# X-PLUG/Youku-mPLUG

Measured on NVIDIA H100. Metric: video-text samples/sec (pretrain 1.3B, 8f x 224^2), higher is better.
Workload: dtype bf16

## Files before the change

### youku-mplug_b200/csrc/gemm_wgmma.cu

```cuda
#include <cuda.h>

#include "common.h"
#include "philox.cuh"
#include "ptx.cuh"
#include "wgmma.cuh"

namespace ymp {

constexpr int BM = 128;
constexpr int BK = 64;
constexpr int WGMMA_K = 16;
constexpr int GEMM_THREADS = 3 * 128;
constexpr int A_STAGE_BYTES = BM * BK * 2;

struct GemmKParams {
  void* D;
  const __nv_bfloat16* bias;
  const void* residual;
  __nv_bfloat16* aux_out;
  const __nv_bfloat16* aux_in;
  int M, N, K;
  int ldd, ldr;
  int a_mn, b_mn;
  int act, out_f32, accumulate, split_k;
  int kb_per_split;
  int res_row_mod;
  int d_row_block, d_row_stride;
  int res_f32;
  int n_fast;
  float alpha;
  int im2col_T, im2col_N, im2col_Wp;
  DropSpec drop;
  int has_drop;
};

template <int BN>
struct GemmCfg {
  static constexpr int NSTAGE = (BN == 256) ? 4 : 6;
  static constexpr int B_STAGE_BYTES = BN * BK * 2;
  static constexpr int STAGE_BYTES = A_STAGE_BYTES + B_STAGE_BYTES;
  static constexpr int STG_LD = BN + 4;
  static_assert(BM * STG_LD * 4 <= NSTAGE * STAGE_BYTES, "epilogue staging reuses the operand ring");
  static constexpr int SMEM_BYTES = NSTAGE * STAGE_BYTES + 256 + 1024;
};

template <int BN>
struct EpiCfg {
  static constexpr int TPR = BN / 8;
  static constexpr int RPP = 256 / TPR;
  static constexpr int GROUP = 4;
  static_assert(BM % (RPP * GROUP) == 0, "row groups tile BM");
};

__device__ __forceinline__ uint2 ld_bf16x4(const __nv_bfloat16* p) { return __ldg(reinterpret_cast<const uint2*>(p)); }
__device__ __forceinline__ void st_bf16x4(__nv_bfloat16* p, const float* f) {
  *reinterpret_cast<uint2*>(p) = make_uint2(pack_bf16(f[0], f[1]), pack_bf16(f[2], f[3]));
}

struct EpiIn {
  uint32_t res[8];
  uint32_t aux[4];
};
__device__ __forceinline__ void epilogue_fetch(const GemmKParams& p, int row, const int (&col)[2], bool full, EpiIn& in) {
  if (row >= p.M || !full) return;
  if (p.aux_in) {
#pragma unroll
    for (int q = 0; q < 2; ++q) {
      const uint2 a = ld_bf16x4(p.aux_in + (size_t)row * p.ldd + col[q]);
      in.aux[2 * q] = a.x; in.aux[2 * q + 1] = a.y;
    }
  }
  if (p.residual) {
    const int rrow = p.res_row_mod ? row % p.res_row_mod : row;
#pragma unroll
    for (int q = 0; q < 2; ++q) {
      if (p.res_f32) {
        const float4 a = __ldg(reinterpret_cast<const float4*>(reinterpret_cast<const float*>(p.residual) + (size_t)rrow * p.ldr + col[q]));
        in.res[4 * q] = __float_as_uint(a.x); in.res[4 * q + 1] = __float_as_uint(a.y);
        in.res[4 * q + 2] = __float_as_uint(a.z); in.res[4 * q + 3] = __float_as_uint(a.w);
      } else {
        const uint2 a = ld_bf16x4(reinterpret_cast<const __nv_bfloat16*>(p.residual) + (size_t)rrow * p.ldr + col[q]);
        in.res[2 * q] = a.x; in.res[2 * q + 1] = a.y;
      }
    }
  }
}

template <bool DROP>
__device__ __forceinline__ void epilogue_row(const GemmKParams& p, float (&v)[8], int row, const int (&col)[2], bool full,
                                             const uint32_t (&bias)[4], const EpiIn& in, const DropState& ds) {
  if (row >= p.M) return;
  const int drow = p.d_row_block ? (row / p.d_row_block) * p.d_row_stride + row % p.d_row_block : row;
  const int rrow = p.res_row_mod ? row % p.res_row_mod : row;
  if (p.alpha != 1.0f) {
#pragma unroll
    for (int i = 0; i < 8; ++i) v[i] = v[i] * p.alpha;
  }

  if (full) {
    if (p.bias) {
#pragma unroll
      for (int i = 0; i < 4; ++i) { v[2 * i] += bf16_lo(bias[i]); v[2 * i + 1] += bf16_hi(bias[i]); }
    }
    const size_t off[2] = {(size_t)row * p.ldd + col[0], (size_t)row * p.ldd + col[1]};
    const size_t doff[2] = {(size_t)drow * p.ldd + col[0], (size_t)drow * p.ldd + col[1]};
    if (p.aux_in) {
#pragma unroll
      for (int i = 0; i < 4; ++i) { v[2 * i] *= bf16_lo(in.aux[i]); v[2 * i + 1] *= bf16_hi(in.aux[i]); }
    } else if (p.act == YMP_ACT_GELU_ERF) {
      if (p.aux_out) {
        float x[8], d[8];
#pragma unroll
        for (int i = 0; i < 8; ++i) x[i] = v[i];
        gelu_erf_both_x8(x, v, d);
        st_bf16x4(p.aux_out + off[0], d);
        st_bf16x4(p.aux_out + off[1], d + 4);
      } else {
        float x[8];
#pragma unroll
        for (int i = 0; i < 8; ++i) x[i] = v[i];
        gelu_erf_x8(x, v);
      }
    } else if (p.act == YMP_ACT_GELU_TANH) {
      if (p.aux_out) {
        float d[8];
#pragma unroll
        for (int i = 0; i < 8; ++i) v[i] = gelu_tanh_both(v[i], d[i]);
        st_bf16x4(p.aux_out + off[0], d);
        st_bf16x4(p.aux_out + off[1], d + 4);
      } else {
#pragma unroll
        for (int i = 0; i < 8; ++i) v[i] = gelu_tanh(v[i]);
      }
    } else if (p.aux_out) {
      st_bf16x4(p.aux_out + off[0], v);
      st_bf16x4(p.aux_out + off[1], v + 4);
    }
    if constexpr (DROP) {
#pragma unroll
      for (int q = 0; q < 2; ++q) drop4(ds, (uint32_t)row, (uint32_t)col[q], v[4 * q], v[4 * q + 1], v[4 * q + 2], v[4 * q + 3]);
    }
    if (p.residual) {
      if (p.res_f32) {
#pragma unroll
        for (int i = 0; i < 8; ++i) v[i] += __uint_as_float(in.res[i]);
      } else {
#pragma unroll
        for (int i = 0; i < 4; ++i) { v[2 * i] += bf16_lo(in.res[i]); v[2 * i + 1] += bf16_hi(in.res[i]); }
      }
    }
#pragma unroll
    for (int q = 0; q < 2; ++q) {
      if (!p.out_f32) {
        st_bf16x4(reinterpret_cast<__nv_bfloat16*>(p.D) + doff[q], v + 4 * q);
      } else if (!p.accumulate) {
        *reinterpret_cast<float4*>(reinterpret_cast<float*>(p.D) + doff[q]) = make_float4(v[4 * q], v[4 * q + 1], v[4 * q + 2], v[4 * q + 3]);
      } else {
        asm volatile("red.global.add.v4.f32 [%0], {%1, %2, %3, %4};" ::"l"(reinterpret_cast<float*>(p.D) + doff[q]),
                     "f"(v[4 * q]), "f"(v[4 * q + 1]), "f"(v[4 * q + 2]), "f"(v[4 * q + 3])
                     : "memory");
      }
    }
  } else {
#pragma unroll
    for (int i = 0; i < 8; ++i) {
      const int c = col[i >> 2] + (i & 3);
      if (c < p.N) {
        float x = v[i];
        if (p.bias) x += __bfloat162float(p.bias[c]);
        const size_t off = (size_t)row * p.ldd + c, doff = (size_t)drow * p.ldd + c;
        if (p.aux_in) {
          x *= __bfloat162float(p.aux_in[off]);
        } else if (p.act == YMP_ACT_GELU_ERF) {
          float d; x = gelu_erf_both(x, d);
          if (p.aux_out) p.aux_out[off] = __float2bfloat16(d);
        } else if (p.act == YMP_ACT_GELU_TANH) {
          float d; x = gelu_tanh_both(x, d);
          if (p.aux_out) p.aux_out[off] = __float2bfloat16(d);
        } else if (p.aux_out) {
          p.aux_out[off] = __float2bfloat16(x);
        }
        if constexpr (DROP) {
          const uint4 w = drop_words(ds, (uint32_t)row, (uint32_t)c >> 2);
          const uint32_t wc = (c & 3) == 0 ? w.x : (c & 3) == 1 ? w.y : (c & 3) == 2 ? w.z : w.w;
          x = wc >= ds.thresh ? x * ds.scale : 0.f;
        }
        if (p.residual)
          x += p.res_f32 ? reinterpret_cast<const float*>(p.residual)[(size_t)rrow * p.ldr + c]
                         : __bfloat162float(reinterpret_cast<const __nv_bfloat16*>(p.residual)[(size_t)rrow * p.ldr + c]);
        if (!p.out_f32) reinterpret_cast<__nv_bfloat16*>(p.D)[doff] = __float2bfloat16(x);
        else if (!p.accumulate) reinterpret_cast<float*>(p.D)[doff] = x;
        else atomicAdd(reinterpret_cast<float*>(p.D) + doff, x);
      }
    }
  }
}

constexpr int IM2COL_SUB_BYTES = BM * 32;
__device__ __forceinline__ void load_a_im2col(uint8_t* sa, const CUtensorMap* tma, uint64_t* bar, int m0, int kb,
                                              const GemmKParams& p) {
  const int T = p.im2col_T, c = kb >> 2, y0 = (kb & 3) * 4;
  const int pt = m0 / T;
  for (int i = 0; i < BM / T; ++i) {
    const int g = pt + i, b = g / p.im2col_N, n = g - b * p.im2col_N;
    const int ny = n / p.im2col_Wp, nx = n - ny * p.im2col_Wp;
#pragma unroll
    for (int ks = 0; ks < 4; ++ks) {
      uint8_t* dst = sa + ks * IM2COL_SUB_BYTES + i * T * 32;
      tma_load_5d(dst, tma, bar, nx * 16, ny * 16 + y0 + ks, 0, c, b);
    }
  }
}
__device__ __forceinline__ void named_sync(int id, int n) { asm volatile("bar.sync %0, %1;" ::"r"(id), "r"(n) : "memory"); }

template <int BN, int AMN, int BMN>
__global__ void __launch_bounds__(GEMM_THREADS, 1)
gemm_bf16_wgmma_kernel(const __grid_constant__ CUtensorMap tma_a, const __grid_constant__ CUtensorMap tma_b,
                       const GemmKParams p) {
  using Cfg = GemmCfg<BN>;
  constexpr int NSTAGE = Cfg::NSTAGE;
  extern __shared__ uint8_t smem_raw[];
  const uint32_t raw_addr = smem_u32(smem_raw);
  uint8_t* smem = smem_raw + ((1024u - (raw_addr & 1023u)) & 1023u);
  uint8_t* smem_a = smem;
  uint8_t* smem_b = smem + NSTAGE * A_STAGE_BYTES;
  uint64_t* full_bar = reinterpret_cast<uint64_t*>(smem + NSTAGE * Cfg::STAGE_BYTES);
  uint64_t* empty_bar = full_bar + NSTAGE;

  const int wg = threadIdx.x >> 7;
  const int num_m = (p.M + BM - 1) / BM;
  const int num_n = (p.N + BN - 1) / BN;
  const int kb_total = (p.K + BK - 1) / BK;
  const int ks = blockIdx.x % p.split_k;
  const int t = blockIdx.x / p.split_k;
  const int m_blk = p.n_fast ? t / num_n : t % num_m;
  const int n_blk = p.n_fast ? t % num_n : t / num_m;
  const int kb0 = ks * p.kb_per_split;
  const int kb1 = min(kb_total, kb0 + p.kb_per_split);

  if (threadIdx.x == 0) {
    tma_prefetch_desc(&tma_a);
    tma_prefetch_desc(&tma_b);
    for (int i = 0; i < NSTAGE; ++i) {
      mbar_init(&full_bar[i], 1);
      mbar_init(&empty_bar[i], 2);
    }
    fence_mbar_init();
  }
  __syncthreads();

  if (wg == 0) {
    if (threadIdx.x == 0) {
      int stage = 0;
      uint32_t phase = 0;
      for (int kb = kb0; kb < kb1; ++kb) {
        mbar_wait(&empty_bar[stage], phase ^ 1);
        mbar_expect_tx(&full_bar[stage], Cfg::STAGE_BYTES);
        uint8_t* sa = smem_a + stage * A_STAGE_BYTES;
        uint8_t* sb = smem_b + stage * Cfg::B_STAGE_BYTES;
        if (p.im2col_T) {
          load_a_im2col(sa, &tma_a, &full_bar[stage], m_blk * BM, kb, p);
        } else if (!AMN) {
          tma_load_2d(sa, &tma_a, &full_bar[stage], kb * BK, m_blk * BM);
        } else {
#pragma unroll
          for (int c = 0; c < BM / 64; ++c)
            tma_load_2d(sa + c * (64 * BK * 2), &tma_a, &full_bar[stage], m_blk * BM + c * 64, kb * BK);
        }
        if (!BMN) {
          tma_load_2d(sb, &tma_b, &full_bar[stage], kb * BK, n_blk * BN);
        } else {
#pragma unroll
          for (int c = 0; c < BN / 64; ++c)
            tma_load_2d(sb + c * (64 * BK * 2), &tma_b, &full_bar[stage], n_blk * BN + c * 64, kb * BK);
        }
        if (++stage == NSTAGE) { stage = 0; phase ^= 1; }
      }
    }
    return;
  }

  const int cw = wg - 1;
  float acc[BN / 2];
#pragma unroll
  for (int i = 0; i < BN / 2; ++i) acc[i] = 0.f;
  {
    int stage = 0;
    uint32_t phase = 0;
    int prev = -1;
    wgmma_fence_acc(acc);
    for (int kb = kb0; kb < kb1; ++kb) {
      mbar_wait(&full_bar[stage], phase);
      const uint32_t sa = smem_u32(smem_a + stage * A_STAGE_BYTES);
      const uint32_t sb = smem_u32(smem_b + stage * Cfg::B_STAGE_BYTES);
      wgmma_fence();
#pragma unroll
      for (int k = 0; k < BK / WGMMA_K; ++k) {
        const uint64_t da = p.im2col_T ? make_smem_desc(sa + k * IM2COL_SUB_BYTES + cw * 64 * 32, 16, 256, 3)
                            : AMN ? make_smem_desc(sa + cw * 8192 + k * WGMMA_K * 128, 64 * BK * 2, 1024, 1)
                                  : make_smem_desc(sa + cw * 8192 + k * WGMMA_K * 2, 16, 1024, 1);
        const uint64_t db = BMN ? make_smem_desc(sb + k * WGMMA_K * 128, 64 * BK * 2, 1024, 1)
                                : make_smem_desc(sb + k * WGMMA_K * 2, 16, 1024, 1);
        if constexpr (BN == 256) wgmma_m64n256<AMN, BMN>(acc, da, db, 1u);
        else wgmma_m64n128<AMN, BMN>(acc, da, db, 1u);
      }
      wgmma_commit();
      wgmma_wait<1>();
      if (prev >= 0 && (threadIdx.x & 127) == 0) mbar_arrive(&empty_bar[prev]);
      prev = stage;
      if (++stage == NSTAGE) { stage = 0; phase ^= 1; }
    }
    wgmma_wait<0>();
    wgmma_fence_acc(acc);
  }

  named_sync(1, 256);
  float* stg = reinterpret_cast<float*>(smem);
  {
    const int lt = threadIdx.x & 127, r0 = cw * 64 + (lt >> 5) * 16 + ((lt & 31) >> 2), c0 = 2 * (lt & 3);
#pragma unroll
    for (int j = 0; j < BN / 8; ++j) {
      *reinterpret_cast<float2*>(stg + r0 * Cfg::STG_LD + 8 * j + c0) = make_float2(acc[4 * j], acc[4 * j + 1]);
      *reinterpret_cast<float2*>(stg + (r0 + 8) * Cfg::STG_LD + 8 * j + c0) = make_float2(acc[4 * j + 2], acc[4 * j + 3]);
    }
  }
  named_sync(1, 256);
  DropState ds;
  if (p.has_drop) ds = drop_state(p.drop);
  using Epi = EpiCfg<BN>;
  const int et = threadIdx.x - 128, tj = et % Epi::TPR, tr = et / Epi::TPR;
  const int col[2] = {n_blk * BN + 4 * tj, n_blk * BN + BN / 2 + 4 * tj};
  const bool full = col[1] + 4 <= p.N;
  uint32_t bias[4];
  if (p.bias && full) {
#pragma unroll
    for (int q = 0; q < 2; ++q) {
      const uint2 b = ld_bf16x4(p.bias + col[q]);
      bias[2 * q] = b.x; bias[2 * q + 1] = b.y;
    }
  }
#pragma unroll 1
  for (int lr0 = tr; lr0 < BM; lr0 += Epi::RPP * Epi::GROUP) {
    EpiIn in[Epi::GROUP];
#pragma unroll
    for (int u = 0; u < Epi::GROUP; ++u) epilogue_fetch(p, m_blk * BM + lr0 + u * Epi::RPP, col, full, in[u]);
#pragma unroll
    for (int u = 0; u < Epi::GROUP; ++u) {
      const int lr = lr0 + u * Epi::RPP;
      const float4 a = *reinterpret_cast<const float4*>(stg + lr * Cfg::STG_LD + 4 * tj);
      const float4 b = *reinterpret_cast<const float4*>(stg + lr * Cfg::STG_LD + BN / 2 + 4 * tj);
      float v[8] = {a.x, a.y, a.z, a.w, b.x, b.y, b.z, b.w};
      if (p.has_drop) epilogue_row<true>(p, v, m_blk * BM + lr, col, full, bias, in[u], ds);
      else epilogue_row<false>(p, v, m_blk * BM + lr, col, full, bias, in[u], ds);
    }
  }
}

typedef CUresult (*EncodeTiledFn)(CUtensorMap*, CUtensorMapDataType, cuuint32_t, void*,
                                  const cuuint64_t*, const cuuint64_t*, const cuuint32_t*,
                                  const cuuint32_t*, CUtensorMapInterleave, CUtensorMapSwizzle,
                                  CUtensorMapL2promotion, CUtensorMapFloatOOBfill);

static EncodeTiledFn get_encode_fn() {
  static EncodeTiledFn fn = nullptr;
  static bool tried = false;
  if (!tried) {
    tried = true;
    void* f = nullptr;
    cudaDriverEntryPointQueryResult q;
    if (cudaGetDriverEntryPoint("cuTensorMapEncodeTiled", &f, cudaEnableDefault, &q) == cudaSuccess &&
        q == cudaDriverEntryPointSuccess)
      fn = reinterpret_cast<EncodeTiledFn>(f);
    else
      cudaGetLastError();
  }
  return fn;
}

static int make_map(CUtensorMap* m, const void* ptr, uint64_t inner, uint64_t outer, uint64_t ld,
                    uint32_t box_inner, uint32_t box_outer) {
  EncodeTiledFn fn = get_encode_fn();
  if (!fn) return set_error(YMP_ECUDA, "cuTensorMapEncodeTiled entry point unavailable (no driver?)");
  cuuint64_t dims[2] = {inner, outer};
  cuuint64_t strides[1] = {ld * 2};
  cuuint32_t box[2] = {box_inner, box_outer};
  cuuint32_t estr[2] = {1, 1};
  CUresult r = fn(m, CU_TENSOR_MAP_DATA_TYPE_BFLOAT16, 2, const_cast<void*>(ptr), dims, strides, box,
                  estr, CU_TENSOR_MAP_INTERLEAVE_NONE, CU_TENSOR_MAP_SWIZZLE_128B,
                  CU_TENSOR_MAP_L2_PROMOTION_L2_256B, CU_TENSOR_MAP_FLOAT_OOB_FILL_NONE);
  if (r != CUDA_SUCCESS)
    return set_error(YMP_ECUDA, "cuTensorMapEncodeTiled failed (%d): inner=%llu outer=%llu ld=%llu",
                     (int)r, (unsigned long long)inner, (unsigned long long)outer,
                     (unsigned long long)ld);
  return YMP_OK;
}

static int make_video_map(CUtensorMap* m, const ymp_gemm_args* a) {
  EncodeTiledFn fn = get_encode_fn();
  if (!fn) return set_error(YMP_ECUDA, "cuTensorMapEncodeTiled entry point unavailable (no driver?)");
  const cuuint64_t W = a->im2col_W, H = a->im2col_H, T = a->im2col_T, C = a->im2col_C, B = a->im2col_B;
  cuuint64_t dims[5] = {W, H, T, C, B};
  cuuint64_t strides[4] = {W * 2, H * W * 2, T * H * W * 2, C * T * H * W * 2};
  cuuint32_t box[5] = {16, 1, (cuuint32_t)T, 1, 1};
  cuuint32_t estr[5] = {1, 1, 1, 1, 1};
  CUresult r = fn(m, CU_TENSOR_MAP_DATA_TYPE_BFLOAT16, 5, const_cast<void*>(a->A), dims, strides, box, estr,
                  CU_TENSOR_MAP_INTERLEAVE_NONE, CU_TENSOR_MAP_SWIZZLE_32B, CU_TENSOR_MAP_L2_PROMOTION_L2_256B,
                  CU_TENSOR_MAP_FLOAT_OOB_FILL_NONE);
  if (r != CUDA_SUCCESS) return set_error(YMP_ECUDA, "cuTensorMapEncodeTiled (video, 5-D) failed (%d)", (int)r);
  return YMP_OK;
}

template <int BN, int AMN, int BMN>
static int launch_gemm_t(const CUtensorMap& ta, const CUtensorMap& tb, const GemmKParams& kp, int grid, cudaStream_t stream) {
  using Cfg = GemmCfg<BN>;
  static DeviceOnce once;
  if (once.first())
    YMP_CUDA(cudaFuncSetAttribute(gemm_bf16_wgmma_kernel<BN, AMN, BMN>, cudaFuncAttributeMaxDynamicSharedMemorySize,
                                  Cfg::SMEM_BYTES));
  gemm_bf16_wgmma_kernel<BN, AMN, BMN><<<grid, GEMM_THREADS, Cfg::SMEM_BYTES, stream>>>(ta, tb, kp);
  YMP_LAUNCH_CHECK();
  return YMP_OK;
}

template <int BN>
static int launch_gemm(const ymp_gemm_args* a, const GemmKParams& kp, cudaStream_t stream) {
  CUtensorMap ta, tb;
  int rc;
  if (a->im2col_P) rc = make_video_map(&ta, a);
  else if (!a->a_mn_major) rc = make_map(&ta, a->A, a->K, a->M, a->lda, BK, BM);
  else rc = make_map(&ta, a->A, a->M, a->K, a->lda, 64, BK);
  if (rc) return rc;
  if (!a->b_mn_major) rc = make_map(&tb, a->B, a->K, a->N, a->ldb, BK, BN);
  else rc = make_map(&tb, a->B, a->N, a->K, a->ldb, 64, BK);
  if (rc) return rc;
  const int num_m = (a->M + BM - 1) / BM, num_n = (a->N + BN - 1) / BN;
  const int grid = num_m * num_n * kp.split_k;
  switch (kp.a_mn * 2 + kp.b_mn) {
    case 0: return launch_gemm_t<BN, 0, 0>(ta, tb, kp, grid, stream);
    case 1: return launch_gemm_t<BN, 0, 1>(ta, tb, kp, grid, stream);
    case 2: return launch_gemm_t<BN, 1, 0>(ta, tb, kp, grid, stream);
    default: return launch_gemm_t<BN, 1, 1>(ta, tb, kp, grid, stream);
  }
}

}

extern "C" int ymp_gemm(const ymp_gemm_args* a, void* stream) {
  using namespace ymp;
  YMP_CHECK_ARG(a != nullptr, "ymp_gemm: null args");
  YMP_CHECK_ARG(a->A && a->B && a->D, "ymp_gemm: null A/B/D");
  YMP_CHECK_ARG(a->M > 0 && a->N > 0 && a->K > 0, "ymp_gemm: bad shape M=%d N=%d K=%d", a->M, a->N, a->K);
  if (a->im2col_P) {
    const int P = a->im2col_P, T = a->im2col_T;
    YMP_CHECK_ARG(P == 16 && T > 0 && T % 8 == 0 && 128 % T == 0 && a->im2col_H % P == 0 && a->im2col_W % P == 0 && !a->a_mn_major,
                  "ymp_gemm(im2col): needs P = 16, T %% 8 == 0, 128 %% T == 0, H, W multiples of P (P=%d T=%d H=%d W=%d)", P, T,
                  a->im2col_H, a->im2col_W);
    const long rows = (long)a->im2col_B * (a->im2col_H / P) * (a->im2col_W / P) * T;
    YMP_CHECK_ARG(a->M == rows && a->K == a->im2col_C * P * P, "ymp_gemm(im2col): needs M = B*N*T, K = C*P*P (M=%d K=%d)", a->M, a->K);
  }
  const bool ia = a->im2col_P != 0;
  YMP_CHECK_ARG((ia || a->lda % 8 == 0) && a->ldb % 8 == 0, "ymp_gemm: lda/ldb must be multiples of 8 (lda=%d ldb=%d)", a->lda, a->ldb);
  YMP_CHECK_ARG(aligned16(a->A) && aligned16(a->B) && aligned16(a->D), "ymp_gemm: A/B/D must be 16-byte aligned");
  YMP_CHECK_ARG(ia || a->lda >= (a->a_mn_major ? a->M : a->K), "ymp_gemm: lda too small");
  YMP_CHECK_ARG(a->ldb >= (a->b_mn_major ? a->N : a->K), "ymp_gemm: ldb too small");
  YMP_CHECK_ARG(a->ldd >= a->N && a->ldd % 8 == 0, "ymp_gemm: ldd must be >= N and a multiple of 8 (ldd=%d)", a->ldd);
  YMP_CHECK_ARG(a->act >= 0 && a->act <= 2, "ymp_gemm: bad act %d", a->act);
  YMP_CHECK_ARG(!a->residual || (a->ldr >= a->N && a->ldr % 8 == 0 && aligned16(a->residual)), "ymp_gemm: bad residual ld/alignment");
  YMP_CHECK_ARG(a->residual_dtype == YMP_DT_BF16 || a->residual_dtype == YMP_DT_F32, "ymp_gemm: bad residual_dtype");
  YMP_CHECK_ARG(!a->bias || aligned16(a->bias), "ymp_gemm: bias must be 16-byte aligned");
  YMP_CHECK_ARG(!a->aux_out || aligned16(a->aux_out), "ymp_gemm: aux_out alignment");
  YMP_CHECK_ARG(!a->aux_in || aligned16(a->aux_in), "ymp_gemm: aux_in alignment");
  YMP_CHECK_ARG(!(a->accumulate && a->out_dtype != YMP_DT_F32), "ymp_gemm: accumulate needs fp32 output");
  YMP_CHECK_ARG(!(a->accumulate && (a->bias || a->aux_out || a->aux_in || a->act || a->residual)),
                "ymp_gemm: accumulate mode supports only alpha and bias-free linear epilogue");
  YMP_CHECK_ARG(a->res_row_mod >= 0 && a->d_row_block >= 0 && (a->d_row_block == 0 || a->d_row_stride >= a->d_row_block),
                "ymp_gemm: bad res_row_mod / d_row_block / d_row_stride");
  YMP_CHECK_ARG(!(a->drop.rng && a->drop.p > 0.f) || (a->drop.p < 1.f && !a->aux_out && !a->accumulate),
                "ymp_gemm: dropout needs 0 < p < 1 and is not combined with aux_out / accumulate");
  YMP_CHECK_ARG(a->tile_n == 0 || a->tile_n == 128 || a->tile_n == 256 || a->tile_n == 512,
                "ymp_gemm: tile_n must be 0 (auto), 128, 256 or 512 (the widest tile: 256 columns on sm_90)");

  const int kb_total = (a->K + BK - 1) / BK;
  const int sms = num_sms();
  int bn = a->tile_n == 512 ? 256 : a->tile_n;
  if (a->im2col_P && bn == 0) bn = (a->N <= 128) ? 128 : 256;
  if (bn == 0) {
    const long t256 = (long)((a->M + BM - 1) / BM) * ((a->N + 255) / 256);
    bn = (a->N <= 128 || (t256 < sms && a->split_k <= 1 && !a->accumulate)) ? 128 : 256;
  }
  int split = a->split_k;
  if (split <= 0) {
    split = 1;
    if (a->accumulate) {
      const long tiles = (long)((a->M + BM - 1) / BM) * ((a->N + bn - 1) / bn);
      const long workers = sms;
      long best = -1;
      for (int sp = 1; sp <= 64 && sp * 8 <= kb_total; ++sp) {
        const long waves = (tiles * sp + workers - 1) / workers;
        const long cost = waves * ((kb_total + sp - 1) / sp + 24);
        if (best < 0 || cost < best) { best = cost; split = sp; }
      }
    }
  }
  YMP_CHECK_ARG(split == 1 || (a->accumulate && a->out_dtype == YMP_DT_F32), "ymp_gemm: split_k>1 needs accumulate=1 and fp32 output");
  if (split > kb_total) split = kb_total;
  int per = (kb_total + split - 1) / split;
  split = (kb_total + per - 1) / per;

  GemmKParams kp;
  kp.D = a->D;
  kp.bias = reinterpret_cast<const __nv_bfloat16*>(a->bias);
  kp.residual = a->residual;
  kp.res_f32 = (a->residual_dtype == YMP_DT_F32) ? 1 : 0;
  kp.aux_out = reinterpret_cast<__nv_bfloat16*>(a->aux_out);
  kp.aux_in = reinterpret_cast<const __nv_bfloat16*>(a->aux_in);
  kp.M = a->M; kp.N = a->N; kp.K = a->K;
  kp.ldd = a->ldd; kp.ldr = a->ldr;
  kp.a_mn = a->a_mn_major ? 1 : 0; kp.b_mn = a->b_mn_major ? 1 : 0;
  kp.act = a->act; kp.out_f32 = (a->out_dtype == YMP_DT_F32); kp.accumulate = a->accumulate ? 1 : 0;
  kp.split_k = split; kp.kb_per_split = per;
  kp.alpha = a->alpha;
  kp.n_fast = ((long)a->M >= (long)a->N) ? 1 : 0;
  kp.res_row_mod = a->res_row_mod; kp.d_row_block = a->d_row_block; kp.d_row_stride = a->d_row_stride;
  kp.im2col_T = a->im2col_P ? a->im2col_T : 0;
  kp.im2col_Wp = a->im2col_P ? a->im2col_W / a->im2col_P : 0;
  kp.im2col_N = a->im2col_P ? (a->im2col_H / a->im2col_P) * kp.im2col_Wp : 0;
  kp.has_drop = (a->drop.rng && a->drop.p > 0.f) ? 1 : 0;
  kp.drop.rng = a->drop.rng; kp.drop.site = a->drop.site; kp.drop.p = a->drop.p;
  cudaStream_t st = reinterpret_cast<cudaStream_t>(stream);
  if (bn == 256) return launch_gemm<256>(a, kp, st);
  return launch_gemm<128>(a, kp, st);
}
```

### youku-mplug_b200/csrc/ptx.cuh

```cuda
#pragma once
#include <cuda_bf16.h>
#include <cuda_runtime.h>
#include <stdint.h>

namespace ymp {

__device__ __forceinline__ uint32_t smem_u32(const void* p) {
  return static_cast<uint32_t>(__cvta_generic_to_shared(p));
}

__device__ __forceinline__ bool elect_one() {
  uint32_t pred = 0;
  asm volatile(
      "{\n\t.reg .pred P;\n\t"
      "elect.sync _|P, 0xffffffff;\n\t"
      "selp.u32 %0, 1, 0, P;\n\t}\n"
      : "=r"(pred));
  return pred != 0;
}

__device__ __forceinline__ void mbar_init(uint64_t* bar, uint32_t count) {
  asm volatile("mbarrier.init.shared::cta.b64 [%0], %1;" ::"r"(smem_u32(bar)), "r"(count));
}
__device__ __forceinline__ void fence_mbar_init() {
  asm volatile("fence.mbarrier_init.release.cluster;" ::: "memory");
}
__device__ __forceinline__ void fence_proxy_async() {
  asm volatile("fence.proxy.async.shared::cta;" ::: "memory");
}
__device__ __forceinline__ void mbar_expect_tx(uint64_t* bar, uint32_t bytes) {
  asm volatile("mbarrier.arrive.expect_tx.shared::cta.b64 _, [%0], %1;" ::"r"(smem_u32(bar)),
               "r"(bytes)
               : "memory");
}
__device__ __forceinline__ void mbar_arrive(uint64_t* bar) {
  asm volatile("mbarrier.arrive.shared::cta.b64 _, [%0];" ::"r"(smem_u32(bar)) : "memory");
}
__device__ __forceinline__ bool mbar_try_wait(uint64_t* bar, uint32_t parity) {
  uint32_t ok;
  asm volatile(
      "{\n\t.reg .pred P;\n\t"
      "mbarrier.try_wait.parity.shared::cta.b64 P, [%1], %2;\n\t"
      "selp.u32 %0, 1, 0, P;\n\t}\n"
      : "=r"(ok)
      : "r"(smem_u32(bar)), "r"(parity)
      : "memory");
  return ok != 0;
}
__device__ __forceinline__ void mbar_wait(uint64_t* bar, uint32_t parity) {
  while (!mbar_try_wait(bar, parity)) {
  }
}

__device__ __forceinline__ void tma_prefetch_desc(const void* desc) {
  asm volatile("prefetch.tensormap [%0];" ::"l"(reinterpret_cast<uint64_t>(desc)) : "memory");
}
__device__ __forceinline__ void tma_load_2d(void* smem_dst, const void* desc, uint64_t* bar,
                                            int32_t c0, int32_t c1) {
  asm volatile(
      "cp.async.bulk.tensor.2d.shared::cluster.global.mbarrier::complete_tx::bytes"
      " [%0], [%1, {%3, %4}], [%2];"
      :
      : "r"(smem_u32(smem_dst)), "l"(reinterpret_cast<uint64_t>(desc)), "r"(smem_u32(bar)),
        "r"(c0), "r"(c1)
      : "memory");
}

__device__ __forceinline__ void tma_load_5d(void* smem_dst, const void* desc, uint64_t* bar, int32_t c0, int32_t c1,
                                            int32_t c2, int32_t c3, int32_t c4) {
  asm volatile(
      "cp.async.bulk.tensor.5d.shared::cluster.global.mbarrier::complete_tx::bytes"
      " [%0], [%1, {%3, %4, %5, %6, %7}], [%2];"
      :
      : "r"(smem_u32(smem_dst)), "l"(reinterpret_cast<uint64_t>(desc)), "r"(smem_u32(bar)), "r"(c0), "r"(c1), "r"(c2),
        "r"(c3), "r"(c4)
      : "memory");
}
__device__ __forceinline__ void cp_async16(void* smem, const void* gmem) {
  asm volatile("cp.async.cg.shared.global [%0], [%1], 16;" ::"r"(smem_u32(smem)), "l"(gmem) : "memory");
}
__device__ __forceinline__ void cp_async_commit() { asm volatile("cp.async.commit_group;" ::: "memory"); }
template <int N>
__device__ __forceinline__ void cp_async_wait() {
  asm volatile("cp.async.wait_group %0;" ::"n"(N) : "memory");
}
__device__ __forceinline__ void ldsm_x4(uint32_t (&r)[4], uint32_t addr) {
  asm volatile("ldmatrix.sync.aligned.m8n8.x4.shared.b16 {%0,%1,%2,%3}, [%4];"
               : "=r"(r[0]), "=r"(r[1]), "=r"(r[2]), "=r"(r[3]) : "r"(addr));
}
__device__ __forceinline__ void ldsm_x4_t(uint32_t (&r)[4], uint32_t addr) {
  asm volatile("ldmatrix.sync.aligned.m8n8.x4.trans.shared.b16 {%0,%1,%2,%3}, [%4];"
               : "=r"(r[0]), "=r"(r[1]), "=r"(r[2]), "=r"(r[3]) : "r"(addr));
}
__device__ __forceinline__ void mma16816(float (&c)[4], const uint32_t (&a)[4], uint32_t b0, uint32_t b1) {
  asm volatile(
      "mma.sync.aligned.m16n8k16.row.col.f32.bf16.bf16.f32 {%0,%1,%2,%3}, {%4,%5,%6,%7}, {%8,%9}, "
      "{%0,%1,%2,%3};"
      : "+f"(c[0]), "+f"(c[1]), "+f"(c[2]), "+f"(c[3])
      : "r"(a[0]), "r"(a[1]), "r"(a[2]), "r"(a[3]), "r"(b0), "r"(b1));
}

__device__ __forceinline__ void wgmma_fence() { asm volatile("wgmma.fence.sync.aligned;" ::: "memory"); }
__device__ __forceinline__ void wgmma_commit() { asm volatile("wgmma.commit_group.sync.aligned;" ::: "memory"); }
template <int N>
__device__ __forceinline__ void wgmma_wait() { asm volatile("wgmma.wait_group.sync.aligned %0;" ::"n"(N) : "memory"); }
template <int N>
__device__ __forceinline__ void wgmma_fence_acc(float (&d)[N]) {
#pragma unroll
  for (int i = 0; i < N; ++i) asm volatile("" : "+f"(d[i])::"memory");
}

__device__ __forceinline__ uint64_t make_smem_desc(uint32_t saddr, uint32_t lbo_bytes, uint32_t sbo_bytes, uint32_t layout) {
  uint64_t d = 0;
  d |= (uint64_t)((saddr & 0x3FFFF) >> 4);
  d |= (uint64_t)((lbo_bytes >> 4) & 0x3FFF) << 16;
  d |= (uint64_t)((sbo_bytes >> 4) & 0x3FFF) << 32;
  d |= (uint64_t)layout << 62;
  return d;
}

__device__ __forceinline__ void griddep_wait() { asm volatile("griddepcontrol.wait;" ::: "memory"); }
__device__ __forceinline__ void griddep_launch() { asm volatile("griddepcontrol.launch_dependents;" ::: "memory"); }
__device__ __forceinline__ uint4 ld_nc_v4(const uint4* p) {
  uint4 v;
  asm("ld.global.nc.L1::no_allocate.v4.u32 {%0, %1, %2, %3}, [%4];" : "=r"(v.x), "=r"(v.y), "=r"(v.z), "=r"(v.w) : "l"(p));
  return v;
}
__device__ __forceinline__ float bf16_lo(uint32_t v) { return __uint_as_float(v << 16); }
__device__ __forceinline__ float bf16_hi(uint32_t v) { return __uint_as_float(v & 0xFFFF0000u); }
__device__ __forceinline__ uint32_t pack_bf16(float lo, float hi) {
  __nv_bfloat162 t = __floats2bfloat162_rn(lo, hi);
  return *reinterpret_cast<uint32_t*>(&t);
}

__device__ __forceinline__ float fast_erf(float x) {
  float ax = fabsf(x);
  float t = __fdividef(1.0f, fmaf(0.3275911f, ax, 1.0f));
  float poly = fmaf(fmaf(fmaf(fmaf(1.061405429f, t, -1.453152027f), t, 1.421413741f), t,
                         -0.284496736f),
                    t, 0.254829592f) *
               t;
  float r = 1.0f - poly * __expf(-ax * ax);
  return copysignf(r, x);
}
__device__ __forceinline__ float tanh_fast(float x) {
  float y;
  asm("tanh.approx.f32 %0, %1;" : "=f"(y) : "f"(x));
  return y;
}
constexpr float PHI_ZERO_X = -4.5000081062316895f;
__device__ __forceinline__ float norm_cdf_pdf(float x, float& pdf) {
  const float xc = fminf(fmaxf(x, PHI_ZERO_X), 4.5f);
  const float xx = x * x;
  const float u = fminf(xx, 20.25f);
  float e;
  asm("ex2.approx.ftz.f32 %0, %1;" : "=f"(e) : "f"(fmaf(xx, -0.72134752044f, -1.32574806474f)));
  pdf = e;
  float q = -1.6543631001e-12f;
  q = fmaf(q, u, 1.9532824653e-10f);
  q = fmaf(q, u, -1.0287317553e-08f);
  q = fmaf(q, u, 3.2170341066e-07f);
  q = fmaf(q, u, -6.7323919166e-06f);
  q = fmaf(q, u, 1.0108823657e-04f);
  q = fmaf(q, u, -1.1397043329e-03f);
  q = fmaf(q, u, 9.8841767687e-03f);
  q = fmaf(q, u, -6.6411978624e-02f);
  q = fmaf(q, u, 3.9892175804e-01f);
  return fmaf(xc, q, 0.5f);
}
__device__ __forceinline__ float gelu_erf(float x) {
  float e;
  return x * norm_cdf_pdf(x, e);
// ... 104 lines not shown
```

Measured before the change: 154.7.

## Add persistent ping-pong WGMMA GEMM with per-warpgroup epilogue overlap

Adds a persistent GEMM kernel for non-accumulating GEMMs with K up to 1024 and no aux input. It launches one CTA per SM, and the two consumer warpgroups alternate whole 128x128 tiles, each computing the full 128 rows with two m64n128 accumulators. A turn barrier hands the mainloop to the other warpgroup, so one tile's epilogue overlaps the next tile's MMAs. It also uses setmaxnreg to move registers from the producer to the consumers, stages the epilogue through dedicated buffers in 64-column passes, and moves tile scheduling into a shared host/device plan. In exchange it uses fewer pipeline stages, fixes the tile at BN=128, and runs a more complex barrier protocol with some risk of register pressure or spills at 232 registers.

Result: no change. 156.0 (median of 6 runs) (+0.8%).

```diff
diff --git a/youku-mplug_b200/csrc/gemm_sched.h b/youku-mplug_b200/csrc/gemm_sched.h
--- /dev/null
+++ b/youku-mplug_b200/csrc/gemm_sched.h
@@ -0,0 +1,73 @@
+#pragma once
+#include <stdint.h>
+
+#if defined(__CUDACC__)
+#define YMP_HD __host__ __device__ __forceinline__
+#else
+#define YMP_HD inline
+#endif
+
+namespace ymp {
+
+constexpr int GEMM_BM = 128;
+constexpr int GEMM_BN = 128;
+constexpr int GEMM_BK = 64;
+constexpr int GEMM_NSTAGE = 4;
+
+struct GemmGrid {
+  int num_m, num_n;
+  int kb_total;
+  int split_k;
+  int kb_per_split;
+  int n_fast;
+  int units;
+  int ctas;
+};
+
+struct GemmUnit {
+  int m_blk, n_blk, kb0, kb1;
+};
+
+YMP_HD GemmUnit gemm_unit(const GemmGrid& g, int u) {
+  const int ks = u % g.split_k, t = u / g.split_k;
+  GemmUnit r;
+  r.m_blk = g.n_fast ? t / g.num_n : t % g.num_m;
+  r.n_blk = g.n_fast ? t % g.num_n : t / g.num_m;
+  r.kb0 = ks * g.kb_per_split;
+  r.kb1 = r.kb0 + g.kb_per_split < g.kb_total ? r.kb0 + g.kb_per_split : g.kb_total;
+  return r;
+}
+
+YMP_HD int ring_stage(uint32_t it) { return (int)(it % GEMM_NSTAGE); }
+YMP_HD uint32_t ring_phase(uint32_t it) { return (it / GEMM_NSTAGE) & 1u; }
+
+YMP_HD uint32_t turn_parity(int j) { return (uint32_t)((j - 1) >> 1) & 1u; }
+
+YMP_HD int gemm_auto_split(long tiles, int kb_total, int sms, int overhead) {
+  int split = 1;
+  long best = -1;
+  for (int sp = 1; sp <= 64 && sp * 8 <= kb_total; ++sp) {
+    const long rounds = (tiles * sp + sms - 1) / sms;
+    const long cost = rounds * ((kb_total + sp - 1) / sp + overhead);
+    if (best < 0 || cost < best) { best = cost; split = sp; }
+  }
+  return split;
+}
+
+YMP_HD GemmGrid gemm_plan(int M, int N, int K, int split_req, int accumulate, int sms, int bn, int persistent) {
+  GemmGrid g;
+  g.num_m = (M + GEMM_BM - 1) / GEMM_BM;
+  g.num_n = (N + bn - 1) / bn;
+  g.kb_total = (K + GEMM_BK - 1) / GEMM_BK;
+  int split = split_req;
+  if (split <= 0) split = accumulate ? gemm_auto_split((long)g.num_m * g.num_n, g.kb_total, sms, 24) : 1;
+  if (split > g.kb_total) split = g.kb_total;
+  g.kb_per_split = (g.kb_total + split - 1) / split;
+  g.split_k = (g.kb_total + g.kb_per_split - 1) / g.kb_per_split;
+  g.n_fast = M >= N ? 1 : 0;
+  g.units = g.num_m * g.num_n * g.split_k;
+  g.ctas = persistent && sms < g.units ? sms : g.units;
+  return g;
+}
+
+}
diff --git a/youku-mplug_b200/csrc/gemm_wgmma.cu b/youku-mplug_b200/csrc/gemm_wgmma.cu
--- a/youku-mplug_b200/csrc/gemm_wgmma.cu
+++ b/youku-mplug_b200/csrc/gemm_wgmma.cu
@@ -1,17 +1,28 @@
 #include <cuda.h>
 
 #include "common.h"
+#include "gemm_sched.h"
 #include "philox.cuh"
 #include "ptx.cuh"
 #include "wgmma.cuh"
 
 namespace ymp {
 
-constexpr int BM = 128;
-constexpr int BK = 64;
+constexpr int BM = GEMM_BM;
+constexpr int BN = GEMM_BN;
+constexpr int BK = GEMM_BK;
+constexpr int NSTAGE = GEMM_NSTAGE;
 constexpr int WGMMA_K = 16;
 constexpr int GEMM_THREADS = 3 * 128;
 constexpr int A_STAGE_BYTES = BM * BK * 2;
+constexpr int B_STAGE_BYTES = BN * BK * 2;
+constexpr int STAGE_BYTES = A_STAGE_BYTES + B_STAGE_BYTES;
+constexpr int EPI_COLS = 64;
+constexpr int STG_LD = EPI_COLS + 4;
+constexpr int STG_BYTES = BM * STG_LD * 4;
+constexpr int SMEM_BYTES = NSTAGE * STAGE_BYTES + 2 * STG_BYTES + 256 + 1024;
+static_assert(SMEM_BYTES <= 227 * 1024, "ring + two staging buffers fit one SM");
+constexpr int PRODUCER_REGS = 40, CONSUMER_REGS = 232;
 
 struct GemmKParams {
   void* D;
@@ -22,33 +33,20 @@
   int M, N, K;
   int ldd, ldr;
   int a_mn, b_mn;
-  int act, out_f32, accumulate, split_k;
-  int kb_per_split;
+  int act, out_f32, accumulate;
   int res_row_mod;
   int d_row_block, d_row_stride;
   int res_f32;
-  int n_fast;
   float alpha;
   int im2col_T, im2col_N, im2col_Wp;
   DropSpec drop;
   int has_drop;
 };
 
-template <int BN>
-struct GemmCfg {
-  static constexpr int NSTAGE = (BN == 256) ? 4 : 6;
-  static constexpr int B_STAGE_BYTES = BN * BK * 2;
-  static constexpr int STAGE_BYTES = A_STAGE_BYTES + B_STAGE_BYTES;
-  static constexpr int STG_LD = BN + 4;
-  static_assert(BM * STG_LD * 4 <= NSTAGE * STAGE_BYTES, "epilogue staging reuses the operand ring");
-  static constexpr int SMEM_BYTES = NSTAGE * STAGE_BYTES + 256 + 1024;
-};
-
-template <int BN>
 struct EpiCfg {
-  static constexpr int TPR = BN / 8;
-  static constexpr int RPP = 256 / TPR;
-  static constexpr int GROUP = 4;
+  static constexpr int TPR = EPI_COLS / 8;
+  static constexpr int RPP = 128 / TPR;
+  static constexpr int GROUP = 2;
   static_assert(BM % (RPP * GROUP) == 0, "row groups tile BM");
 };
 
@@ -213,11 +211,198 @@
 }
 __device__ __forceinline__ void named_sync(int id, int n) { asm volatile("bar.sync %0, %1;" ::"r"(id), "r"(n) : "memory"); }
 
+template <int PASS>
+__device__ __forceinline__ void stage_pass(float* stg, const float (&acc)[2][64], int lt) {
+  const int r0 = (lt >> 5) * 16 + ((lt & 31) >> 2), c0 = 2 * (lt & 3);
+#pragma unroll
+  for (int h = 0; h < 2; ++h) {
+#pragma unroll
+    for (int j = 0; j < EPI_COLS / 8; ++j) {
+      const int a = 4 * (PASS * (EPI_COLS / 8) + j);
+      *reinterpret_cast<float2*>(stg + (64 * h + r0) * STG_LD + 8 * j + c0) = make_float2(acc[h][a], acc[h][a + 1]);
+      *reinterpret_cast<float2*>(stg + (64 * h + r0 + 8) * STG_LD + 8 * j + c0) = make_float2(acc[h][a + 2], acc[h][a + 3]);
+    }
+  }
+}
+
+template <int AMN, int BMN>
+__global__ void __launch_bounds__(GEMM_THREADS, 1)
+gemm_bf16_wgmma_kernel(const __grid_constant__ CUtensorMap tma_a, const __grid_constant__ CUtensorMap tma_b,
+                       const GemmKParams p, const GemmGrid g) {
+  extern __shared__ uint8_t smem_raw[];
+  const uint32_t raw_addr = smem_u32(smem_raw);
+  uint8_t* smem = smem_raw + ((1024u - (raw_addr & 1023u)) & 1023u);
+  uint8_t* smem_a = smem;
+  uint8_t* smem_b = smem + NSTAGE * A_STAGE_BYTES;
+  float* stg_all = reinterpret_cast<float*>(smem + NSTAGE * STAGE_BYTES);
+  uint64_t* full_bar = reinterpret_cast<uint64_t*>(smem + NSTAGE * STAGE_BYTES + 2 * STG_BYTES);
+  uint64_t* empty_bar = full_bar + NSTAGE;
+  uint64_t* turn_bar = empty_bar + NSTAGE;
+
+  const int wg = threadIdx.x >> 7;
+  if (threadIdx.x == 0) {
+    tma_prefetch_desc(&tma_a);
+    tma_prefetch_desc(&tma_b);
+    for (int i = 0; i < NSTAGE; ++i) {
+      mbar_init(&full_bar[i], 1);
+      mbar_init(&empty_bar[i], 1);
+    }
+    mbar_init(&turn_bar[0], 1);
+    mbar_init(&turn_bar[1], 1);
+    fence_mbar_init();
+  }
+  __syncthreads();
+
+  if (wg == 0) {
+    setmaxnreg_dec<PRODUCER_REGS>();
+    if (threadIdx.x == 0) {
+      uint32_t it = 0;
+      for (int u = blockIdx.x; u < g.units; u += gridDim.x) {
+        const GemmUnit w = gemm_unit(g, u);
+        for (int kb = w.kb0; kb < w.kb1; ++kb, ++it) {
+          const int stage = ring_stage(it);
+          mbar_wait(&empty_bar[stage], ring_phase(it) ^ 1);
+          mbar_expect_tx(&full_bar[stage], STAGE_BYTES);
+          uint8_t* sa = smem_a + stage * A_STAGE_BYTES;
+          uint8_t* sb = smem_b + stage * B_STAGE_BYTES;
+          if (p.im2col_T) {
+            load_a_im2col(sa, &tma_a, &full_bar[stage], w.m_blk * BM, kb, p);
+          } else if (!AMN) {
+            tma_load_2d(sa, &tma_a, &full_bar[stage], kb * BK, w.m_blk * BM);
+          } else {
+#pragma unroll
+            for (int c = 0; c < BM / 64; ++c)
+              tma_load_2d(sa + c * (64 * BK * 2), &tma_a, &full_bar[stage], w.m_blk * BM + c * 64, kb * BK);
+          }
+          if (!BMN) {
+            tma_load_2d(sb, &tma_b, &full_bar[stage], kb * BK, w.n_blk * BN);
+          } else {
+#pragma unroll
+            for (int c = 0; c < BN / 64; ++c)
+              tma_load_2d(sb + c * (64 * BK * 2), &tma_b, &full_bar[stage], w.n_blk * BN + c * 64, kb * BK);
+          }
+        }
+      }
+    }
+    return;
+  }
+
+  setmaxnreg_inc<CONSUMER_REGS>();
+  const int cw = wg - 1, lt = threadIdx.x & 127;
+  float* stg = stg_all + cw * (BM * STG_LD);
+  DropState ds;
+  if (p.has_drop) ds = drop_state(p.drop);
+  const int tj = lt % EpiCfg::TPR, tr = lt / EpiCfg::TPR;
+  float acc[2][64];
+  uint32_t it = 0;
+  int j = 0;
+  for (int u = blockIdx.x; u < g.units; u += gridDim.x, ++j) {
+    const GemmUnit w = gemm_unit(g, u);
+    if ((j & 1) != cw) {
+      it += w.kb1 - w.kb0;
+      continue;
+    }
+#pragma unroll
+    for (int h = 0; h < 2; ++h)
+#pragma unroll
+      for (int i = 0; i < 64; ++i) acc[h][i] = 0.f;
+    if (j > 0) mbar_wait(&turn_bar[cw], turn_parity(j));
+    int prev = -1;
+    wgmma_fence_acc(acc[0]);
+    wgmma_fence_acc(acc[1]);
+    for (int kb = w.kb0; kb < w.kb1; ++kb, ++it) {
+      const int stage = ring_stage(it);
+      mbar_wait(&full_bar[stage], ring_phase(it));
+      const uint32_t sa = smem_u32(smem_a + stage * A_STAGE_BYTES);
+      const uint32_t sb = smem_u32(smem_b + stage * B_STAGE_BYTES);
+      wgmma_fence();
+#pragma unroll
+      for (int k = 0; k < BK / WGMMA_K; ++k) {
+        const uint64_t db = BMN ? make_smem_desc(sb + k * WGMMA_K * 128, 64 * BK * 2, 1024, 1)
+                                : make_smem_desc(sb + k * WGMMA_K * 2, 16, 1024, 1);
+#pragma unroll
+        for (int h = 0; h < 2; ++h) {
+          const uint64_t da = p.im2col_T ? make_smem_desc(sa + k * IM2COL_SUB_BYTES + h * 64 * 32, 16, 256, 3)
+                              : AMN ? make_smem_desc(sa + h * 8192 + k * WGMMA_K * 128, 64 * BK * 2, 1024, 1)
+                                    : make_smem_desc(sa + h * 8192 + k * WGMMA_K * 2, 16, 1024, 1);
+          wgmma_m64n128<AMN, BMN>(acc[h], da, db, 1u);
+        }
+      }
+      wgmma_commit();
+      wgmma_wait<1>();
+      if (prev >= 0 && lt == 0) mbar_arrive(&empty_bar[prev]);
+      prev = stage;
+    }
+    if (lt == 0) mbar_arrive(&turn_bar[cw ^ 1]);
+    wgmma_wait<0>();
+    wgmma_fence_acc(acc[0]);
+    wgmma_fence_acc(acc[1]);
+    if (lt == 0) mbar_arrive(&empty_bar[prev]);
+
+    static_assert(BN / EPI_COLS <= 4, "stage_pass dispatch");
+#pragma unroll
+    for (int pass = 0; pass < BN / EPI_COLS; ++pass) {
+      named_sync(1 + cw, 128);
+      switch (pass) {
+        case 0: stage_pass<0>(stg, acc, lt); break;
+        case 1: stage_pass<1>(stg, acc, lt); break;
+        case 2: if constexpr (BN / EPI_COLS > 2) stage_pass<2>(stg, acc, lt); break;
+        default: if constexpr (BN / EPI_COLS > 3) stage_pass<3>(stg, acc, lt); break;
+      }
+      named_sync(1 + cw, 128);
+      const int n0 = w.n_blk * BN + pass * EPI_COLS;
+      const int col[2] = {n0 + 4 * tj, n0 + EPI_COLS / 2 + 4 * tj};
+      const bool full = col[1] + 4 <= p.N;
+      uint32_t bias[4];
+      if (p.bias && full) {
+#pragma unroll
+        for (int q = 0; q < 2; ++q) {
+          const uint2 b = ld_bf16x4(p.bias + col[q]);
+          bias[2 * q] = b.x; bias[2 * q + 1] = b.y;
+        }
+      }
+#pragma unroll 1
+      for (int lr0 = tr; lr0 < BM; lr0 += EpiCfg::RPP * EpiCfg::GROUP) {
+        EpiIn in[EpiCfg::GROUP];
+#pragma unroll
+        for (int v = 0; v < EpiCfg::GROUP; ++v) epilogue_fetch(p, w.m_blk * BM + lr0 + v * EpiCfg::RPP, col, full, in[v]);
+#pragma unroll
+        for (int v = 0; v < EpiCfg::GROUP; ++v) {
+          const int lr = lr0 + v * EpiCfg::RPP;
+          const float4 a = *reinterpret_cast<const float4*>(stg + lr * STG_LD + 4 * tj);
+          const float4 b = *reinterpret_cast<const float4*>(stg + lr * STG_LD + EPI_COLS / 2 + 4 * tj);
+          float x[8] = {a.x, a.y, a.z, a.w, b.x, b.y, b.z, b.w};
+          if (p.has_drop) epilogue_row<true>(p, x, w.m_blk * BM + lr, col, full, bias, in[v], ds);
+          else epilogue_row<false>(p, x, w.m_blk * BM + lr, col, full, bias, in[v], ds);
+        }
+      }
+    }
+  }
+}
+
+template <int BN>
+struct TileCfg {
+  static constexpr int NSTAGE = (BN == 256) ? 4 : 6;
+  static constexpr int B_BYTES = BN * BK * 2;
+  static constexpr int STAGE_BYTES = A_STAGE_BYTES + B_BYTES;
+  static constexpr int STG_LD = BN + 4;
+  static_assert(BM * STG_LD * 4 <= NSTAGE * STAGE_BYTES, "epilogue staging reuses the operand ring");
+  static constexpr int SMEM_BYTES = NSTAGE * STAGE_BYTES + 256 + 1024;
+};
+
+template <int BN>
+struct TileEpiCfg {
+  static constexpr int TPR = BN / 8;
+  static constexpr int RPP = 256 / TPR;
+  static constexpr int GROUP = 4;
+  static_assert(BM % (RPP * GROUP) == 0, "row groups tile BM");
+};
+
 template <int BN, int AMN, int BMN>
 __global__ void __launch_bounds__(GEMM_THREADS, 1)
-gemm_bf16_wgmma_kernel(const __grid_constant__ CUtensorMap tma_a, const __grid_constant__ CUtensorMap tma_b,
-                       const GemmKParams p) {
-  using Cfg = GemmCfg<BN>;
+gemm_bf16_tile_kernel(const __grid_constant__ CUtensorMap tma_a, const __grid_constant__ CUtensorMap tma_b,
+                       const GemmKParams p, const GemmGrid g) {
+  using Cfg = TileCfg<BN>;
   constexpr int NSTAGE = Cfg::NSTAGE;
   extern __shared__ uint8_t smem_raw[];
   const uint32_t raw_addr = smem_u32(smem_raw);
@@ -228,15 +413,8 @@
   uint64_t* empty_bar = full_bar + NSTAGE;
 
   const int wg = threadIdx.x >> 7;
-  const int num_m = (p.M + BM - 1) / BM;
-  const int num_n = (p.N + BN - 1) / BN;
-  const int kb_total = (p.K + BK - 1) / BK;
-  const int ks = blockIdx.x % p.split_k;
-  const int t = blockIdx.x / p.split_k;
-  const int m_blk = p.n_fast ? t / num_n : t % num_m;
-  const int n_blk = p.n_fast ? t % num_n : t / num_m;
-  const int kb0 = ks * p.kb_per_split;
-  const int kb1 = min(kb_total, kb0 + p.kb_per_split);
+  const GemmUnit w = gemm_unit(g, blockIdx.x);
+  const int m_blk = w.m_blk, n_blk = w.n_blk, kb0 = w.kb0, kb1 = w.kb1;
 
   if (threadIdx.x == 0) {
     tma_prefetch_desc(&tma_a);
@@ -257,7 +435,7 @@
         mbar_wait(&empty_bar[stage], phase ^ 1);
         mbar_expect_tx(&full_bar[stage], Cfg::STAGE_BYTES);
         uint8_t* sa = smem_a + stage * A_STAGE_BYTES;
-        uint8_t* sb = smem_b + stage * Cfg::B_STAGE_BYTES;
+        uint8_t* sb = smem_b + stage * Cfg::B_BYTES;
         if (p.im2col_T) {
           load_a_im2col(sa, &tma_a, &full_bar[stage], m_blk * BM, kb, p);
         } else if (!AMN) {
@@ -292,7 +470,7 @@
     for (int kb = kb0; kb < kb1; ++kb) {
       mbar_wait(&full_bar[stage], phase);
       const uint32_t sa = smem_u32(smem_a + stage * A_STAGE_BYTES);
-      const uint32_t sb = smem_u32(smem_b + stage * Cfg::B_STAGE_BYTES);
+      const uint32_t sb = smem_u32(smem_b + stage * Cfg::B_BYTES);
       wgmma_fence();
 #pragma unroll
       for (int k = 0; k < BK / WGMMA_K; ++k) {
@@ -327,7 +505,7 @@
   named_sync(1, 256);
   DropState ds;
   if (p.has_drop) ds = drop_state(p.drop);
-  using Epi = EpiCfg<BN>;
+  using Epi = TileEpiCfg<BN>;
   const int et = threadIdx.x - 128, tj = et % Epi::TPR, tr = et / Epi::TPR;
   const int col[2] = {n_blk * BN + 4 * tj, n_blk * BN + BN / 2 + 4 * tj};
   const bool full = col[1] + 4 <= p.N;
@@ -410,36 +588,54 @@
   return YMP_OK;
 }
 
-template <int BN, int AMN, int BMN>
-static int launch_gemm_t(const CUtensorMap& ta, const CUtensorMap& tb, const GemmKParams& kp, int grid, cudaStream_t stream) {
-  using Cfg = GemmCfg<BN>;
+template <int AMN, int BMN>
+static int launch_persistent_t(const CUtensorMap& ta, const CUtensorMap& tb, const GemmKParams& kp, const GemmGrid& g,
+                               cudaStream_t stream) {
   static DeviceOnce once;
   if (once.first())
-    YMP_CUDA(cudaFuncSetAttribute(gemm_bf16_wgmma_kernel<BN, AMN, BMN>, cudaFuncAttributeMaxDynamicSharedMemorySize,
-                                  Cfg::SMEM_BYTES));
-  gemm_bf16_wgmma_kernel<BN, AMN, BMN><<<grid, GEMM_THREADS, Cfg::SMEM_BYTES, stream>>>(ta, tb, kp);
+    YMP_CUDA(cudaFuncSetAttribute(gemm_bf16_wgmma_kernel<AMN, BMN>, cudaFuncAttributeMaxDynamicSharedMemorySize, SMEM_BYTES));
+  gemm_bf16_wgmma_kernel<AMN, BMN><<<g.ctas, GEMM_THREADS, SMEM_BYTES, stream>>>(ta, tb, kp, g);
   YMP_LAUNCH_CHECK();
   return YMP_OK;
 }
 
-template <int BN>
-static int launch_gemm(const ymp_gemm_args* a, const GemmKParams& kp, cudaStream_t stream) {
+template <int BN, int AMN, int BMN>
+static int launch_tile_t(const CUtensorMap& ta, const CUtensorMap& tb, const GemmKParams& kp, const GemmGrid& g,
+                         cudaStream_t stream) {
+  using Cfg = TileCfg<BN>;
+  static DeviceOnce once;
+  if (once.first())
+    YMP_CUDA(cudaFuncSetAttribute(gemm_bf16_tile_kernel<BN, AMN, BMN>, cudaFuncAttributeMaxDynamicSharedMemorySize,
+                                  Cfg::SMEM_BYTES));
+  gemm_bf16_tile_kernel<BN, AMN, BMN><<<g.ctas, GEMM_THREADS, Cfg::SMEM_BYTES, stream>>>(ta, tb, kp, g);
+  YMP_LAUNCH_CHECK();
+  return YMP_OK;
+}
+
+template <int AMN, int BMN>
+static int launch_layout(const CUtensorMap& ta, const CUtensorMap& tb, const GemmKParams& kp, const GemmGrid& g, int bn,
+                         bool persistent, cudaStream_t stream) {
+  if (persistent) return launch_persistent_t<AMN, BMN>(ta, tb, kp, g, stream);
+  if (bn == 256) return launch_tile_t<256, AMN, BMN>(ta, tb, kp, g, stream);
+  return launch_tile_t<128, AMN, BMN>(ta, tb, kp, g, stream);
+}
+
+static int launch_gemm(const ymp_gemm_args* a, const GemmKParams& kp, const GemmGrid& g, int bn, bool persistent,
+                       cudaStream_t stream) {
   CUtensorMap ta, tb;
   int rc;
   if (a->im2col_P) rc = make_video_map(&ta, a);
   else if (!a->a_mn_major) rc = make_map(&ta, a->A, a->K, a->M, a->lda, BK, BM);
   else rc = make_map(&ta, a->A, a->M, a->K, a->lda, 64, BK);
   if (rc) return rc;
-  if (!a->b_mn_major) rc = make_map(&tb, a->B, a->K, a->N, a->ldb, BK, BN);
+  if (!a->b_mn_major) rc = make_map(&tb, a->B, a->K, a->N, a->ldb, BK, bn);
   else rc = make_map(&tb, a->B, a->N, a->K, a->ldb, 64, BK);
   if (rc) return rc;
-  const int num_m = (a->M + BM - 1) / BM, num_n = (a->N + BN - 1) / BN;
-  const int grid = num_m * num_n * kp.split_k;
   switch (kp.a_mn * 2 + kp.b_mn) {
-    case 0: return launch_gemm_t<BN, 0, 0>(ta, tb, kp, grid, stream);
-    case 1: return launch_gemm_t<BN, 0, 1>(ta, tb, kp, grid, stream);
-    case 2: return launch_gemm_t<BN, 1, 0>(ta, tb, kp, grid, stream);
-    default: return launch_gemm_t<BN, 1, 1>(ta, tb, kp, grid, stream);
+    case 0: return launch_layout<0, 0>(ta, tb, kp, g, bn, persistent, stream);
+    case 1: return launch_layout<0, 1>(ta, tb, kp, g, bn, persistent, stream);
+    case 2: return launch_layout<1, 0>(ta, tb, kp, g, bn, persistent, stream);
+    default: return launch_layout<1, 1>(ta, tb, kp, g, bn, persistent, stream);
   }
 }
 
@@ -480,32 +676,19 @@
   YMP_CHECK_ARG(a->tile_n == 0 || a->tile_n == 128 || a->tile_n == 256 || a->tile_n == 512,
                 "ymp_gemm: tile_n must be 0 (auto), 128, 256 or 512 (the widest tile: 256 columns on sm_90)");
 
-  const int kb_total = (a->K + BK - 1) / BK;
+  YMP_CHECK_ARG(a->split_k <= 1 || (a->accumulate && a->out_dtype == YMP_DT_F32),
+                "ymp_gemm: split_k>1 needs accumulate=1 and fp32 output");
   const int sms = num_sms();
-  int bn = a->tile_n == 512 ? 256 : a->tile_n;
-  if (a->im2col_P && bn == 0) bn = (a->N <= 128) ? 128 : 256;
-  if (bn == 0) {
-    const long t256 = (long)((a->M + BM - 1) / BM) * ((a->N + 255) / 256);
-    bn = (a->N <= 128 || (t256 < sms && a->split_k <= 1 && !a->accumulate)) ? 128 : 256;
-  }
-  int split = a->split_k;
-  if (split <= 0) {
-    split = 1;
-    if (a->accumulate) {
-      const long tiles = (long)((a->M + BM - 1) / BM) * ((a->N + bn - 1) / bn);
-      const long workers = sms;
-      long best = -1;
-      for (int sp = 1; sp <= 64 && sp * 8 <= kb_total; ++sp) {
-        const long waves = (tiles * sp + workers - 1) / workers;
-        const long cost = waves * ((kb_total + sp - 1) / sp + 24);
-        if (best < 0 || cost < best) { best = cost; split = sp; }
-      }
-    }
-  }
-  YMP_CHECK_ARG(split == 1 || (a->accumulate && a->out_dtype == YMP_DT_F32), "ymp_gemm: split_k>1 needs accumulate=1 and fp32 output");
-  if (split > kb_total) split = kb_total;
-  int per = (kb_total + split - 1) / split;
-  split = (kb_total + per - 1) / per;
+  const bool persistent = !a->accumulate && !a->aux_in && a->K <= 1024;
+  int bn = 128;
+  if (!persistent) {
+    bn = a->tile_n == 512 ? 256 : a->tile_n;
+    if (bn == 0) {
+      const long t256 = (long)((a->M + BM - 1) / BM) * ((a->N + 255) / 256);
+      bn = (a->N <= 128 || (t256 < sms && a->split_k <= 1 && !a->accumulate)) ? 128 : 256;
+    }
+  }
+  const GemmGrid g = gemm_plan(a->M, a->N, a->K, a->split_k, a->accumulate ? 1 : 0, sms, bn, persistent ? 1 : 0);
 
   GemmKParams kp;
   kp.D = a->D;
@@ -518,9 +701,7 @@
   kp.ldd = a->ldd; kp.ldr = a->ldr;
   kp.a_mn = a->a_mn_major ? 1 : 0; kp.b_mn = a->b_mn_major ? 1 : 0;
   kp.act = a->act; kp.out_f32 = (a->out_dtype == YMP_DT_F32); kp.accumulate = a->accumulate ? 1 : 0;
-  kp.split_k = split; kp.kb_per_split = per;
   kp.alpha = a->alpha;
-  kp.n_fast = ((long)a->M >= (long)a->N) ? 1 : 0;
   kp.res_row_mod = a->res_row_mod; kp.d_row_block = a->d_row_block; kp.d_row_stride = a->d_row_stride;
   kp.im2col_T = a->im2col_P ? a->im2col_T : 0;
   kp.im2col_Wp = a->im2col_P ? a->im2col_W / a->im2col_P : 0;
@@ -528,6 +709,5 @@
   kp.has_drop = (a->drop.rng && a->drop.p > 0.f) ? 1 : 0;
   kp.drop.rng = a->drop.rng; kp.drop.site = a->drop.site; kp.drop.p = a->drop.p;
   cudaStream_t st = reinterpret_cast<cudaStream_t>(stream);
-  if (bn == 256) return launch_gemm<256>(a, kp, st);
-  return launch_gemm<128>(a, kp, st);
-}
+  return launch_gemm(a, kp, g, bn, persistent, st);
+}
diff --git a/youku-mplug_b200/csrc/ptx.cuh b/youku-mplug_b200/csrc/ptx.cuh
--- a/youku-mplug_b200/csrc/ptx.cuh
+++ b/youku-mplug_b200/csrc/ptx.cuh
@@ -18,6 +18,11 @@
       : "=r"(pred));
   return pred != 0;
 }
+
+template <int N>
+__device__ __forceinline__ void setmaxnreg_inc() { asm volatile("setmaxnreg.inc.sync.aligned.u32 %0;" ::"n"(N)); }
+template <int N>
+__device__ __forceinline__ void setmaxnreg_dec() { asm volatile("setmaxnreg.dec.sync.aligned.u32 %0;" ::"n"(N)); }
 
 __device__ __forceinline__ void mbar_init(uint64_t* bar, uint32_t count) {
   asm volatile("mbarrier.init.shared::cta.b64 [%0], %1;" ::"r"(smem_u32(bar)), "r"(count));
```
